# facebookresearch/NasRec

Hardware: AMD Instinct MI355X
Metric: supernet samples/sec at batch 256 (Criteo-shape), 1/2/4/8 MI355X (higher is better)
Workload: dtype f32

## Files before the change

include/nasrec_hip.h:

```cpp
#ifndef NASREC_HIP_H
#define NASREC_HIP_H

#include <stdint.h>

#ifdef __cplusplus
extern "C" {
#endif

#define NASREC_MAX_SEGS 8
#define NASREC_MAX_TABLES 32
#define NASREC_EMB_DIM 16
#define NASREC_MHA_PARAMS 1696
#define NASREC_MHA_SAVED 36

enum {
  NASREC_AM_KC = 0,
  NASREC_AM_RC = 1,
  NASREC_AM_TOKR = 2,
  NASREC_AM_TOKK = 3
};
enum { NASREC_CM_PLAIN = 0,
       NASREC_CM_TOKJ = 1    };
enum { NASREC_ACT_NONE = 0, NASREC_ACT_RELU = 1, NASREC_ACT_SILU = 2, NASREC_ACT_SIGMOID = 3 };

// ... 566 lines not shown
typedef struct nasrec_act_bwd_desc {
  int32_t kind;
  int32_t mode, R, D;
  int32_t ld_dy, ld_z, ld_dz;
  int32_t act, dims_in_use;
  const float* dy;
  const float* z;
  float* dz;
} nasrec_act_bwd_desc_t;

typedef struct nasrec_stage_desc {
  int32_t kind;
  int32_t B, Fd, Fs;
  float lr;
  int32_t _pad;
  const float* int_src;   float* int_dst;
  const int64_t* cat_src; int64_t* cat_dst;
  const float* y_src;     float* y_dst;
  float* lr_dst;
  nasrec_embed_desc_t gather;
  nasrec_dedup_ids_desc_t dedup_ids;
} nasrec_stage_desc_t;

#define NASREC_WL_MAX_ITEMS 12
#define NASREC_WL_BLOB_BYTES 3680
#define NASREC_WL_REDUCE_DST 16
typedef struct nasrec_wl_item {
  int32_t kind, part, off;
  int32_t first, nblk;
  int32_t geom[3];
} nasrec_wl_item_t;

typedef struct nasrec_wl_reduce {
  int32_t kind, R, C, ld;
  const float* in;
  int32_t ndst, _pad;
  float* dst[NASREC_WL_REDUCE_DST];
  int32_t dst_off[NASREC_WL_REDUCE_DST], dst_len[NASREC_WL_REDUCE_DST];
} nasrec_wl_reduce_t;

typedef struct nasrec_worklist_desc {
  int32_t kind;
  int32_t n;
  int32_t total_blocks;
  int32_t _pad;
  nasrec_wl_item_t item[NASREC_WL_MAX_ITEMS];
  char blob[NASREC_WL_BLOB_BYTES] __attribute__((aligned(16)));
} nasrec_worklist_desc_t;

typedef struct nasrec_worklist_dev_desc {
  int32_t kind;
  int32_t total_blocks;
  int32_t big;
  int32_t _pad;
  uint32_t pf[6], pm[6];
  const nasrec_worklist_desc_t* dev;
} nasrec_worklist_dev_desc_t;
int nasrec_worklist_prepare(const nasrec_worklist_desc_t* w, void* dev_buf, nasrec_worklist_dev_desc_t* out);

enum {
  NASREC_WL_BODY_KIND = 0,
  NASREC_WL_BODY_TILE = 1,
  NASREC_WL_BODY_SECOND_PASS = 2,
  NASREC_WL_BODY_DENSE_SMALL = 3,
  NASREC_WL_BODY_DENSE_SMALL_DX = 4,
  NASREC_WL_BODY_TOKEN_FWD = 5,
  NASREC_WL_BODY_TOKEN_DX = 6
};
typedef struct nasrec_wl_geometry {
  int32_t nblk;
  int32_t geom[3];
  int32_t big;
  int32_t body;
} nasrec_wl_geometry_t;
int nasrec_worklist_item_geometry(int kind, int part, const void* desc, int bytes, nasrec_wl_geometry_t* out);
int nasrec_worklist_set_wide_min(int wide_min);

#define NASREC_PS_MAX_DEPS 8
#define NASREC_PS_REPL 16
#define NASREC_PS_SHARDS 8
#define NASREC_PS_COUNTER_STRIDE 16
#define NASREC_PS_FLAG_STRIDE 32
typedef struct nasrec_persist_item {
  int32_t kind, part, off;
  int32_t first, nblk;
  int32_t geom[3];
  int32_t ndeps;
  int32_t deps[NASREC_PS_MAX_DEPS];
  int32_t _pad[3];
} nasrec_persist_item_t;
// ... 88 lines not shown
```

nasrec_amd/_lib.py:

```python
import ctypes as C
import os

import torch

_HERE = os.path.dirname(os.path.abspath(__file__))
LIB_PATH = os.environ.get("NASREC_HIP_LIB") or os.path.join(_HERE, "lib", "libnasrec_hip.so")

MAX_SEGS = 8
MAX_TABLES = 32
FINAL_HEAD_K, FINAL_HEAD_N = 32, 256
EMB_DIM = 16
MHA_PARAMS = 1696
MHA_SAVED = 36
REDUCE_MAX_DST = 48

AM_KC, AM_RC, AM_TOKR, AM_TOKK = 0, 1, 2, 3
CM_PLAIN, CM_TOKJ = 0, 1
ACT_NONE, ACT_RELU, ACT_SILU, ACT_SIGMOID = 0, 1, 2, 3
TSV_OK, TSV_NEEDS_PYTHON, TSV_BAD_COLUMNS = 0, 1, 2
ACT_BY_NAME = {"identity": ACT_NONE, "relu": ACT_RELU, "silu": ACT_SILU}

(OP_GEMM, OP_EMBED_GATHER, OP_DOT_TRI_FWD, OP_DOT_TRI_BWD, OP_FM_FWD, OP_FM_BWD, OP_MHA_FWD, OP_MHA_BWD, OP_REDUCE_ROWS,
 OP_COPY_SEGS, OP_GATE_BWD, OP_ROWSUM, OP_FINAL_FWD, OP_BCE, OP_FINAL_BWD, OP_EMB_DEDUP, OP_SUMSQ, OP_CLIP_COEF,
 OP_ADAGRAD_DENSE, OP_ADAGRAD_ROWS, OP_MEMSET, OP_LAYERNORM_FWD, OP_LAYERNORM_BWD, OP_ADD_SEGS, OP_SCALE,
# ... 168 lines not shown
    _fields_ = [("kind", i32), ("B", i32), ("Fs", i32), ("cap", i32), ("idx", vp), ("leader", vp), ("order", vp), ("lists", vp), ("counts", vp),
                ("heads", vp)]


class OptReduce2Desc(C.Structure):
    _fields_ = [("kind", i32), ("B", i32), ("Fs", i32), ("cap", i32), ("rank_B", i32), ("row_blocks", i32), ("rank_stride", i64), ("rows", vp),
                ("leader", vp), ("order", vp), ("lists", vp), ("counts", vp), ("heads", vp), ("sumsq_partial", vp), ("sumsq", SumsqDesc)]


class StageDesc(C.Structure):
    _fields_ = [("kind", i32), ("B", i32), ("Fd", i32), ("Fs", i32), ("lr", f32), ("_pad", i32), ("int_src", vp), ("int_dst", vp),
                ("cat_src", vp), ("cat_dst", vp), ("y_src", vp), ("y_dst", vp), ("lr_dst", vp), ("gather", EmbedDesc), ("dedup_ids", DedupIdsDesc)]


class OptReduceDesc(C.Structure):
    _fields_ = [("kind", i32), ("_pad", i32), ("dedup", EmbDedupDesc), ("sumsq", SumsqDesc)]


class OptApplyDesc(C.Structure):
    _fields_ = [("kind", i32), ("dense_blocks", i32), ("clip", ClipCoefDesc), ("dense", AdagradDenseDesc), ("rows", AdagradRowsDesc)]


WL_MAX_ITEMS, WL_BLOB_BYTES, WL_REDUCE_DST = 12, 3680, 16
WL_WHOLE, WL_MAIN, WL_EPI = 0, 1, 2


class WlItem(C.Structure):
    _fields_ = [("kind", i32), ("part", i32), ("off", i32), ("first", i32), ("nblk", i32), ("geom", i32 * 3)]


class WlReduce(C.Structure):
    _fields_ = [("kind", i32), ("R", i32), ("C", i32), ("ld", i32), ("in_", vp), ("ndst", i32), ("_pad", i32), ("dst", vp * WL_REDUCE_DST),
                ("dst_off", i32 * WL_REDUCE_DST), ("dst_len", i32 * WL_REDUCE_DST)]


class WorklistDesc(C.Structure):
    _fields_ = [("kind", i32), ("n", i32), ("total_blocks", i32), ("_pad", i32), ("item", WlItem * WL_MAX_ITEMS),
                ("blob", C.c_char * WL_BLOB_BYTES)]


(WL_BODY_KIND, WL_BODY_TILE, WL_BODY_SECOND_PASS, WL_BODY_DENSE_SMALL, WL_BODY_DENSE_SMALL_DX, WL_BODY_TOKEN_FWD,
 WL_BODY_TOKEN_DX) = range(7)


class WlGeometry(C.Structure):
    _fields_ = [("nblk", i32), ("geom", i32 * 3), ("big", i32), ("body", i32)]


class WorklistDevDesc(C.Structure):
    _fields_ = [("kind", i32), ("total_blocks", i32), ("big", i32), ("_pad", i32), ("pf", C.c_uint32 * 6), ("pm", C.c_uint32 * 6), ("dev", vp)]


PS_MAX_DEPS, PS_REPL, PS_SHARDS, PS_COUNTER_STRIDE, PS_FLAG_STRIDE = 8, 16, 8, 16, 32


class PersistItem(C.Structure):
    _fields_ = [("kind", i32), ("part", i32), ("off", i32), ("first", i32), ("nblk", i32), ("geom", i32 * 3), ("ndeps", i32),
                ("deps", i32 * PS_MAX_DEPS), ("_pad", i32 * 3)]


class PersistDesc(C.Structure):
    _fields_ = [("kind", i32), ("n", i32), ("total_blocks", i32), ("blob_bytes", i32), ("items", vp), ("blob", vp), ("chunk_item", vp),
                ("counters", vp), ("flags", vp), ("err", vp), ("chunk_cap", i32), ("big", i32), ("trace", vp), ("host_items", vp), ("host_blob", vp)]


# ... 101 lines not shown
    lib.nasrec_worklist_prepare.argtypes = [vp, vp, vp]
    lib.nasrec_worklist_item_geometry.argtypes = [C.c_int, C.c_int, C.c_char_p, C.c_int, C.POINTER(WlGeometry)]
    lib.nasrec_worklist_set_wide_min.argtypes = [C.c_int]
    lib.nasrec_tsv_parse.argtypes = [vp, i64, i32, i32, vp, i64, vp, vp, vp, C.POINTER(i64), C.POINTER(i32)]
    lib.nasrec_tsv_parse.restype = i64
    for name in ("nasrec_gemm", "nasrec_embedding_gather", "nasrec_embedding_dedup", "nasrec_dot_tri", "nasrec_fm",
                 "nasrec_mha_ffn", "nasrec_layernorm", "nasrec_final_logit", "nasrec_bce_logits", "nasrec_adagrad_dense",
                 "nasrec_adagrad_rows", "nasrec_opt_reduce", "nasrec_opt_apply", "nasrec_worklist", "nasrec_dedup_ids", "nasrec_opt_reduce2", "nasrec_final_fused", "nasrec_weight_decay",
                 "nasrec_opt_moments", "nasrec_last_layer_step", "nasrec_roc_auc", "nasrec_weight_ema", "nasrec_decoupled_decay"):
        getattr(lib, name).argtypes = [vp, vp]
    lib.nasrec_roc_auc_workspace_bytes.argtypes = [i64]
    lib.nasrec_roc_auc_workspace_bytes.restype = i64
    lib.nasrec_gemm_route.argtypes = [vp, C.POINTER(C.c_uint)]
    if lib.nasrec_abi_version() != 17:
        raise EngineError("ABI version mismatch: library %d, binding 17" % lib.nasrec_abi_version())
    sizes = (i32 * 45)()
    n = lib.nasrec_desc_sizes(sizes, 45)
    for kind, cls in DESC_BY_KIND.items():
        if kind >= n or sizes[kind] != C.sizeof(cls):
            raise EngineError("struct layout mismatch for op kind %d: library %d bytes, binding %d bytes"
                              % (kind, sizes[kind] if kind < n else -1, C.sizeof(cls)))
    if n <= 37 or sizes[37] != C.sizeof(PersistItem):
        raise EngineError("struct layout mismatch for nasrec_persist_item_t: library %d bytes, binding %d bytes" % (sizes[37] if n > 37 else -1, C.sizeof(PersistItem)))
    _lib = lib
    return lib


def check(rc):
    if rc != 0:
        raise EngineError("nasrec engine error %d: %s" % (rc, _lib.nasrec_last_error().decode(errors="replace")))
```

nasrec_amd/csrc/worklist.hip:

```cpp
#include <stdlib.h>
#include <string.h>

#include <vector>

#include "worklist_body.h"

#define WL_WIDE_MIN_DEFAULT 700
static int& wl_wide_min() {
  static int v = getenv("NASREC_WL_WIDE_MIN") ? atoi(getenv("NASREC_WL_WIDE_MIN")) : WL_WIDE_MIN_DEFAULT;
  return v;
}
extern "C" int nasrec_worklist_set_wide_min(int wide_min) {
  const int prev = wl_wide_min();
  wl_wide_min() = wide_min;
  return prev;
}

static int wl_gemm_geometry(const nasrec_gemm_desc_t* g, nasrec_wl_item_t& it, int blob_left) {
  if (blob_left < (int)offsetof(nasrec_gemm_desc_t, seg)) return nasrec_set_error(-2, "worklist: gemm descriptor head runs past the blob");
  if (g->nseg < 1 || g->nseg > NASREC_MAX_SEGS) return nasrec_set_error(-2, "worklist: gemm nseg=%d", g->nseg);
  const int need = (int)offsetof(nasrec_gemm_desc_t, seg) + g->nseg * (int)sizeof(nasrec_gemm_seg_t);
  if (need > blob_left) return nasrec_set_error(-2, "worklist: truncated gemm descriptor (%d bytes) runs past the blob", need);
  const int nprob = g->zmode ? g->nseg : 1;
  const int S = g->splitk > 1 ? g->splitk : 1;
  if (g->splitk == NASREC_SPLITK_BALANCED) return nasrec_set_error(-2, "worklist: the balanced schedule is a throughput-regime launch");
  if ((it.part == 0) != (S == 1)) return nasrec_set_error(-2, "worklist: gemm part %d with splitk %d", it.part, g->splitk);
  if (S > 1 && !g->workspace) return nasrec_set_error(-3, "worklist: splitk=%d needs a workspace", S);
  int Mmax = 0, Nmax = 0, Kmax = 0;
  long wgs = 0;
  bool aux = false, uniform = true;
  for (int q = 0; q < nprob; ++q) {
    Mmax = g->seg[q].M > Mmax ? g->seg[q].M : Mmax;
    Nmax = g->seg[q].N > Nmax ? g->seg[q].N : Nmax;
    wgs += (long)((g->seg[q].M + 63) / 64) * ((g->seg[q].N + 63) / 64) * S;
  }
  for (int q = 0; q < g->nseg; ++q) {
    const nasrec_gemm_seg_t& s = g->seg[q];
    if (s.A && s.K > Kmax) Kmax = s.K;
    aux = aux || s.Aaux || s.Baux;
    if (!g->zmode && (s.ones_col != g->seg[0].ones_col || s.Mvalid != g->seg[0].Mvalid)) uniform = false;
    if (!g->zmode && s.A && ((s.Aaux != nullptr) != (g->seg[0].Aaux != nullptr) || (s.Baux != nullptr) != (g->seg[0].Baux != nullptr))) uniform = false;
  }
  if (!uniform) return nasrec_set_error(-2, "worklist: k-segments that disagree on row predicates / mask operands take the plain template");
  {
    const bool kca = g->amode == NASREC_AM_KC || g->amode == NASREC_AM_TOKK, kcb = g->bmode == NASREC_AM_KC || g->bmode == NASREC_AM_TOKK;
    if (!kca && kcb) return nasrec_set_error(-2, "worklist: operand binding a=%d b=%d has no body", g->amode, g->bmode);
  }
  if (Mmax <= 0 || Nmax <= 0) {
// ... 480 lines not shown
        if (tid == 0) o2 = __hip_atomic_fetch_add(cnt + NASREC_PS_SHARDS * NASREC_PS_COUNTER_STRIDE, 1ull, __ATOMIC_RELAXED, __HIP_MEMORY_SCOPE_AGENT);
        o2 = ((unsigned long long)__builtin_amdgcn_readfirstlane((unsigned)(o2 >> 32)) << 32) | (unsigned)__builtin_amdgcn_readfirstlane((unsigned)o2);
        last = (o2 + 1) % (unsigned long long)NS == 0;
      }
      if (last && nsucc > 0 && tid < NASREC_PS_REPL)
        __hip_atomic_store(flags + ((size_t)k * NASREC_PS_REPL + tid) * NASREC_PS_FLAG_STRIDE, e1, __ATOMIC_RELAXED, __HIP_MEMORY_SCOPE_AGENT);
    }
  }
  if (trace && tid == 0) trace[4 * (size_t)bid + 3] = wall_clock64();
}

int nasrec_persist_prepare(nasrec_persist_desc_t* d) {
  if (!d || d->kind != NASREC_OP_PERSIST) return nasrec_set_error(-1, "persist: wrong descriptor kind");
  if (d->n < 1 || d->n > 65535) return nasrec_set_error(-2, "persist: n=%d items", d->n);
  if (!d->host_items || !d->host_blob) return nasrec_set_error(-2, "persist: a host table pointer is null");
  const bool dry = !d->items;
  if (!dry && (!d->blob || !d->chunk_item || !d->counters || !d->flags || !d->err)) return nasrec_set_error(-2, "persist: a device table pointer is null");
  std::vector<nasrec_persist_item_t> tab(d->host_items, d->host_items + d->n);
  bool big = false;
  int first = 0;
  for (int k = 0; k < d->n; ++k) {
    nasrec_persist_item_t& p = tab[k];
    if (p.off < 0 || (p.off & 15) || p.off >= d->blob_bytes) return nasrec_set_error(-2, "persist: item %d offset %d", k, p.off);
    if (p.ndeps < 0 || p.ndeps > NASREC_PS_MAX_DEPS) return nasrec_set_error(-2, "persist: item %d has %d dependencies", k, p.ndeps);
    for (int q = 0; q < p.ndeps; ++q)
      if (p.deps[q] < 0 || p.deps[q] >= k) return nasrec_set_error(-2, "persist: item %d depends on item %d (not an earlier one)", k, p.deps[q]);
    nasrec_wl_item_t w;
    w.kind = p.kind, w.part = p.part, w.off = p.off;
    const int rc = wl_item_geometry(w, d->host_blob + p.off, d->blob_bytes - p.off, k, big);
    if (rc) return rc;
    if (w.nblk < 1) return nasrec_set_error(-2, "persist: item %d (kind %d) has no workgroups; the caller drops empty operators", k, p.kind);
    static const int max_wg = getenv("NASREC_PS_MAX_WG") ? atoi(getenv("NASREC_PS_MAX_WG")) : 512;
    const bool tiles = p.kind == NASREC_OP_GEMM && p.part != 2 && (w.geom[2] & 3) != WL_TOKS;
    const bool walks = (p.kind == NASREC_OP_GEMM && p.part == 2) || p.kind == NASREC_OP_FINAL_BWD || tiles;
    const int hint = d->host_items[k]._pad[1];
    const int cap = hint > 0 ? hint : (tiles ? 1 << 30 : max_wg);
    const int upw = walks ? (w.nblk + cap - 1) / (cap > 0 ? cap : 1) : 1;
    const int nwg = (w.nblk + upw - 1) / upw;
    p.first = first, p.nblk = w.nblk;
    p.geom[0] = w.geom[0], p.geom[1] = w.geom[1], p.geom[2] = w.geom[2];
    p._pad[1] = nwg;
    p._pad[2] = ((k + 1 < d->n ? d->host_items[k + 1].off : d->blob_bytes) - p.off + 63) & ~63;
    first += nwg;
  }
  for (int k = 0; k < d->n; ++k) tab[k]._pad[0] = 0;
  for (int k = 0; k < d->n; ++k)
// ... 37 lines not shown
```

nasrec_amd/csrc/worklist_body.h:

```cpp
#pragma once
#include "attention_tok.h"
#include "gemm_rt.h"
#include "final_bodies.h"
#include "interact_bodies.h"
#include "dedup_bodies.h"

#define WL_LDS_BIG_FLOATS 9888
#define WL_LDS_FLOATS 7840
static_assert(MHA_TOK_BWD_LDS_FLOATS <= WL_LDS_BIG_FLOATS && MHA_TOK_FWD_LDS_FLOATS <= WL_LDS_FLOATS, "Transformer bodies fit the worklist launches");

#define WL_TK 64
#ifndef WL_AUX_RING2
#define WL_AUX_RING2 0
#endif
enum { WL_TOKS = 0, WL_T32x32 = 1, WL_T64x16 = 2, WL_T16x64 = 3 };
#define WL_WIDE 32
#define WL_WIDE_TK 32

extern __shared__ __attribute__((aligned(16))) float wl_lds[];

template <typename T>
__device__ __forceinline__ const T& wl_ref(unsigned long long addr) {
  const unsigned lo = __builtin_amdgcn_readfirstlane((unsigned)addr), hi = __builtin_amdgcn_readfirstlane((unsigned)(addr >> 32));
  return *(const T*)(const __attribute__((address_space(4))) T*)(((unsigned long long)hi << 32) | lo);
// ... 306 lines not shown
      for (int j = 0; j < 4; ++j) fx[s][j] = xb[min(16 * s + 4 * fg + j, K - 1) * 16];
#pragma unroll
    for (int s = 0; s < WL_TOKDX_STEPS; ++s)
#pragma unroll
      for (int j = 0; j < 4; ++j) fb[s][j] = fx[s][j] > 0.f ? fb[s][j] : 0.f;
  }
  f32x4 acc = {0.f, 0.f, 0.f, 0.f};
#pragma unroll
  for (int s = 0; s < WL_TOKDX_STEPS; ++s) {
    if (16 * s < K) {
#pragma unroll
      for (int j = 0; j < 4; ++j) {
        const bool in = 16 * s + 4 * fg + j < K;
        acc = __builtin_amdgcn_mfma_f32_16x16x4f32(in ? fa[s][j] : 0.f, in ? fb[s][j] : 0.f, acc, 0, 0, 0);
      }
    }
  }
  {
    const float v4[4] = {acc[0], acc[1], acc[2], acc[3]};
    if (t * 16 + 4 * fg < M) epilogue_store_col4<NASREC_CM_TOKJ>(g, sg, t * 16 + 4 * fg, b * 16 + e, M, v4);
  }
}

__device__ __forceinline__ void wl_gemm_second_pass(unsigned long long blob, int vb_, int per_) {
  const nasrec_gemm_desc_t& g = wl_ref<nasrec_gemm_desc_t>(blob);
  const int vb = __builtin_amdgcn_readfirstlane(vb_), per = __builtin_amdgcn_readfirstlane(per_);
  const int nprob = g.zmode ? g.nseg : 1;
  int Mmax = 0, Nmax = 0;
  for (int q = 0; q < nprob; ++q) {
    Mmax = max(Mmax, g.seg[q].M);
    Nmax = max(Nmax, g.seg[q].N);
  }
  int z = vb / per, v = vb - z * per;
  if (WL_COMPACT_Z && g.zmode) {
    z = 0, v = vb;
    for (; z < nprob - 1; ++z) {
      const int cnt = wl_z_units(g.seg[z].M, g.seg[z].N);
      if (v < cnt) break;
      v -= cnt;
    }
  }
  const long e = (long)v * 256 + threadIdx.x;
  if (g.cmode == NASREC_CM_PLAIN)
    splitk_second_pass<NASREC_CM_PLAIN>(g, Mmax, Nmax, z, e);
  else
    splitk_second_pass<NASREC_CM_TOKJ>(g, Mmax, Nmax, z, e);
}

__device__ __forceinline__ void wl_mha_fwd(unsigned long long blob, int vb) {
  mha_fwd_tok(wl_ref<nasrec_mha_desc_t>(blob), __builtin_amdgcn_readfirstlane(vb), wl_lds);
}

#define WL_PACKED_NONE 0xffffffffu
#define WL_HEAD_BYTES 48
static inline int wl_item_body(int kind, int part, const int32_t (&geom)[3]) {
  if (kind != NASREC_OP_GEMM) return NASREC_WL_BODY_KIND;
  if (part == 2) return NASREC_WL_BODY_SECOND_PASS;
  const int cfg = geom[2];
  if ((cfg & 3) != WL_TOKS) return NASREC_WL_BODY_TILE;
  if (((cfg >> 2) & 3) == 3) return geom[1] == 0 ? NASREC_WL_BODY_DENSE_SMALL_DX : NASREC_WL_BODY_DENSE_SMALL;
  return ((cfg >> 2) & 3) == 1 ? NASREC_WL_BODY_TOKEN_FWD : NASREC_WL_BODY_TOKEN_DX;
}
template <bool BIG>
__device__ __forceinline__ void wl_run(unsigned f01, unsigned f23, unsigned f45, unsigned f67, unsigned f89, unsigned fab, unsigned m01, unsigned m23,
                                       unsigned m45, unsigned m67, unsigned m89, unsigned mab, const unsigned long long base) {
  const nasrec_worklist_desc_t& wl = wl_ref<nasrec_worklist_desc_t>(base);
  float* lds = wl_lds;
  const int bid = blockIdx.x, tid = threadIdx.x, wave = tid >> 6, lane = tid & 63;
  int k = 0, it_first = 0, it_kind, it_part, it_off;
  if (f01 != WL_PACKED_NONE) {
    const unsigned f[6] = {f01, f23, f45, f67, f89, fab}, m[6] = {m01, m23, m45, m67, m89, mab};
    unsigned meta = m01 & 0xffffu;
#pragma unroll
    for (int q = 1; q < NASREC_WL_MAX_ITEMS; ++q) {
      const unsigned fq = (f[q >> 1] >> (16 * (q & 1))) & 0xffffu, mq = (m[q >> 1] >> (16 * (q & 1))) & 0xffffu;
      if ((unsigned)bid >= fq) {
        k = q;
        it_first = (int)fq;
        meta = mq;
      }
    }
    it_kind = meta & 63;
    it_part = (meta >> 6) & 3;
    it_off = (int)(meta >> 8) * 16;
  } else {
#pragma unroll 1
    while (k + 1 < wl.n && bid >= wl.item[k + 1].first) ++k;
    it_first = wl.item[k].first;
    it_kind = wl.item[k].kind;
    it_part = wl.item[k].part;
    it_off = wl.item[k].off;
  }
  const nasrec_wl_item_t& it = wl.item[k];
  const int vb = bid - it_first;
  const unsigned long long blob = base + offsetof(nasrec_worklist_desc_t, blob) + it_off;
  switch (it_kind) {
    case NASREC_OP_GEMM: {
      if (it_part == 2) {
        wl_gemm_second_pass(blob, vb, it.geom[0]);
        break;
      }
      const int cfg = it.geom[2];
      if ((cfg & 3) == WL_TOKS && ((cfg >> 2) & 3) == 3 && it.geom[1] == 0) wl_dense_small_dx(blob, vb, it.geom[0]);
      else if ((cfg & 3) == WL_TOKS && ((cfg >> 2) & 3) == 3) wl_dense_small(blob, vb, it.geom[0], it.geom[1]);
      else if ((cfg & 3) == WL_TOKS && ((cfg >> 2) & 3) == 1) wl_token_fwd(blob, vb, it.geom[0]);
      else if ((cfg & 3) == WL_TOKS) wl_token_dx(blob, vb, it.geom[0]);
      else if ((cfg >> 4) & 1) wl_gemm_bind<true>((cfg >> 2) & 3, cfg & 3, blob, vb, it.geom[0], it.geom[1]);
      else wl_gemm_bind<false>((cfg >> 2) & 3, cfg & (3 | WL_WIDE), blob, vb, it.geom[0], it.geom[1]);
      break;
    }
    case NASREC_OP_MHA_FWD:
      wl_mha_fwd(blob, vb);
      break;
    case NASREC_OP_MHA_BWD:
      if (BIG) mha_bwd_tok(wl_ref<nasrec_mha_desc_t>(blob), __builtin_amdgcn_readfirstlane(vb), wl_lds);
      break;
    case NASREC_OP_FM_FWD: {
      const nasrec_fm_desc_t& d = wl_ref<nasrec_fm_desc_t>(blob);
      const int b = vb * 4 + wave;
      if (b < d.B) fm_fwd_sample(d, b, lane);
      break;
    }
    case NASREC_OP_FM_BWD: {
      const nasrec_fm_desc_t& d = wl_ref<nasrec_fm_desc_t>(blob);
// ... 63 lines not shown
```

nasrec_amd/engine.py:

```python
import copy
import ctypes as C
import json
import math
import os
from typing import Dict, List, Optional

import torch

from . import _lib as L
from . import plan as P
from . import schedule as S
from .optim_spec import OptimSpec

E = 16
DEDUP_SPLIT_MAX_B = min(int(os.environ.get("NASREC_DEDUP_SPLIT_MAX_B", "2048")), L.DEDUP_IDS_MAX_B)
_IDS_AS_ITEM = os.environ.get("NASREC_IDS_AS_ITEM", "1") != "0"
_WL_TUNE = os.environ.get("NASREC_WL_TUNE", "0") == "1"
_WL_TUNE_MARGIN = float(os.environ.get("NASREC_WL_TUNE_MARGIN", "0.004"))
_WL_RESIDENT = os.environ.get("NASREC_WL_RESIDENT", "1") != "0"
_FUSE_FINAL = os.environ.get("NASREC_FUSE_FINAL", "1") != "0"
_FIXED_OPT_TABLE = os.environ.get("NASREC_FIXED_OPT_TABLE", "1") != "0"


def _ptr_array(descs):
# ... 397 lines not shown
            w = ctx.param("_final.weight", (1, K))
            bptr = ctx.param("_final.bias", (1,))
            fd = L.FinalDesc()
            fd.kind = L.OP_FINAL_FWD
            fd.B, fd.nseg = B, len(fsegs)
            fd.w, fd.bias, fd.logits = w, bptr, cp.logits.data_ptr()
            for q, (s, ts) in enumerate(fsegs):
                fd.seg[q], fd.width[q], fd.ld[q], fd.off[q], fd.tok_stride[q] = s.view.ptr, s.width, s.view.ld, s.koff, ts
            ctx.emit(fd)
            if cfg.use_final_sigmoid:
                raise NotImplementedError("use_final_sigmoid is never enabled by the reference CLIs")
            scheduled = self.level_schedule and cfg.fixed and B <= 256
            cp.fwd_levels = cp.bwd_levels = None
            cp.dead_forward = []
            if train:
                if not spec.moments or spec.table_kind:
                    self._ensure_table_state()
                self._build_training_tail(cp, ctx, w, bptr, fsegs, B, K, grad_scale)
            fwd_list = list(ctx.fwd)
            if self.dead_code_elimination and cfg.fixed:
                fwd_list, cp.dead_forward = S.eliminate_dead_forward(fwd_list, ctx.bwd if train else [])
            if scheduled:
                fwd_list = S.order_two_term_accumulates(fwd_list)
                fwd_descs, cp.fwd_levels = S.pack(fwd_list)
                self._resident_worklists(cp, fwd_descs)
            else:
                fwd_descs = fwd_list
            cp.fwd = Program(fwd_descs)
            cp.used_params = list(ctx.used_params)
            if train:
                bd, pre = cp.bce, cp._pre
                fi = next(i for i, dsc in enumerate(ctx.bwd) if isinstance(dsc, L.FinalDesc))
                plain = ctx.bwd[fi]
                assert plain.kind == L.OP_FINAL_BWD
                fused = L.FinalDesc.from_buffer_copy(plain)
                fused.logits, fused.y, fused.loss, fused.dlogits_out = cp.logits.data_ptr(), cp.y.data_ptr(), cp.loss.data_ptr(), cp.dlogits.data_ptr()
                fused.grad_scale = bd.grad_scale
                cp.bce = bd
                bwd_descs = pre[1:] + ctx.bwd[:fi] + [fused] + ctx.bwd[fi + 1:]
                odescs = []
                cp.ids_on_stage = False
                if local_optimizer:
                    odescs = self._optimizer_descs(cp.tail, B, cp.cat_x, sbuf.grad_tensor() if (sbuf.grad_written and not self.host_embedding)
                                                   else None, clip, eps)
                cp.decay0 = cp.tail.decay0 if (local_optimizer and spec.dwd) else None
                ids_in_program = []
                ids = cp.tail.dedup_ids
# ... 5 lines not shown
                        cp.ids_on_stage = True
                    else:
                        odescs = [ids] + odescs
                cp.fb = None
                if scheduled:
                    jf, jb = self._fuse_final(fwd_list, bwd_descs, fused) if _FUSE_FINAL else (fwd_list, bwd_descs)
                    jf, jb = self._fuse_head(jf, jb)
                    fb_descs = None
                    cp.persistent = False
                    cp.level_tuning = None
                    if persist:
                        try:
                            if spec.ema:
                                raise S.PersistRefused("a weight-EMA plan keeps the default launches")
                            fb_descs, cp.fb_levels = S.pack_persistent(
                                ids_in_program + jf + jb, lambda nb: torch.empty(max(int(nb), 16), dtype=torch.uint8, device=self.device),
                                arena.ranges, alloc=ctx.alloc)
                            cp.persistent = True
                            self._persist_errs += [d.err_tensor for d in fb_descs if isinstance(d, L.PersistDesc)]
                        except S.PersistRefused as e:
                            import warnings
                            warnings.warn("persistent step refused (%s): one launch per level instead" % (e,))
                    if fb_descs is None:
                        fb_descs, cp.fb_levels = S.pack(ids_in_program + jf + jb, alloc=ctx.alloc)
                        if _WL_TUNE and S.BALANCE:
                            fb_descs, cp.level_tuning = self._tune_levels(ids_in_program + jf + jb, ctx.alloc, fb_descs)
                    self._resident_worklists(cp, fb_descs)
                    cp.fb = Program(fb_descs)
                    bwd_descs, cp.bwd_levels = S.pack(bwd_descs)
                    self._resident_worklists(cp, bwd_descs)
                cp.bwd = Program(bwd_descs)
                cp.bwd_tail_start = len(pre) - 1 + ctx.bwd_tail_start
                cp.bwd_marks = [(b, len(pre) - 1 + idx) for b, idx in ctx.block_marks]
                cp.bwd_core = Program(pre[1:] + ctx.bwd)
                last = L.FinalDesc.from_buffer_copy(plain)
                for q in range(L.MAX_SEGS):
                    last.dseg[q] = None
                tail = [ctx.bwd[fi + 1]] if plain.nsplit > 1 else []
                cp.bwd_final_only = Program(pre[1:] + [last] + tail)
                cp.opt = Program(odescs)
                if graph:
                    cp.step = Program((cp.fb.descs if cp.fb is not None else cp.fwd.descs + cp.bwd.descs) + cp.opt.descs)
                    cp.step.capture(self.stream.cuda_stream)
            elif graph:
                cp.fwd.capture(self.stream.cuda_stream)
        cp.bf16_launches = P.bf16_launches(cp.fwd.descs) + (P.bf16_launches(cp.bwd.descs) if train else 0)
        cp.bf16_token_launches = P.bf16_token_launches(cp.fwd.descs) + (P.bf16_token_launches(cp.bwd.descs) if train else 0)
        if graph or arena is None or cfg.fixed:
            self.stream.synchronize()
        self._plans[key] = cp
        self._last_plan = (fast, choice, cp)
        return cp
# ... 1022 lines not shown
```

nasrec_amd/schedule.py:

```python
import ctypes as C
import os
from typing import List, Tuple

from . import _lib as L

E = 16
MHA_PARAM_FLOATS = [768, 48, 256, 16, 16, 16, 256, 16, 256, 16, 16, 16]


class Acc:
    __slots__ = ("ptr", "width", "stride", "rows", "end")

    def __init__(self, ptr, rows, width_f, ld_f):
        self.ptr = int(ptr)
        self.rows = max(int(rows), 1)
        self.width = int(width_f) * 4
        self.stride = int(ld_f) * 4 if self.rows > 1 else self.width
        if self.stride < self.width:
            self.stride = self.width
        self.end = self.ptr + (self.rows - 1) * self.stride + self.width


def _flat(ptr, n_floats):
    return Acc(ptr, 1, n_floats, n_floats)
# ... 10 lines not shown


def _operand(ptr, mode, R, K, ld):
    if not ptr:
        return None
    if mode == L.AM_KC:
        return Acc(ptr, R, K, ld)
    if mode == L.AM_RC:
        return Acc(ptr, K, R, ld)
    if mode == L.AM_TOKR:
        return Acc(ptr, (R + 15) // 16, K * E, ld)
    return Acc(ptr, (K + 15) // 16, R * E, ld)


def _cview(ptr, cmode, M, N, ldc):
    if not ptr:
        return None
    if cmode == L.CM_PLAIN:
        return Acc(ptr, M, N, ldc)
    return Acc(ptr, (N + 15) // 16, M * E, ldc)


def _gemm_io(d, part):
    R, W = [], []
    nprob = d.nseg if d.zmode else 1
    S = d.splitk if d.splitk > 1 else 1
    Mm = max(d.seg[q].M for q in range(nprob))
    Nm = max(d.seg[q].N for q in range(nprob))
    ws = _flat(d.workspace, S * Mm * Nm * nprob) if (S > 1 and d.workspace) else None
    if d.splitk == L.SPLITK_BALANCED and d.workspace:
        ws = _flat(d.workspace, L.SK_WORKSPACE_FLOATS)
    if part in ("whole", "main"):
        for q in range(d.nseg):
            s = d.seg[q]
            if not s.A:
                continue
            M, N = (s.M, s.N) if d.zmode else (d.seg[0].M, d.seg[0].N)
            Nb = N - (1 if s.ones_col else 0)
            for ptr, mode, rr, ld in ((s.A, d.amode, M, s.lda), (s.Aaux, d.amode, M, s.lda), (s.B, d.bmode, Nb, s.ldb), (s.Baux, d.bmode, Nb, s.ldb)):
                a = _operand(ptr, mode, rr, s.K, ld)
                if a is not None:
                    R.append(a)
        if part == "main":
            W.append(ws)
            return R, W
        if part == "whole" and ws is not None:
# ... 193 lines not shown

    def __init__(self, desc, part="whole"):
        self.desc, self.part = desc, part
        self.level = 0
        self.index = 0

    def __getattr__(self, name):
        if name in ("reads", "writes"):
            io = desc_io(self.desc, self.part)
            self.reads, self.writes = io if io is not None else (None, None)
        elif name == "item":
            self.item = _item(self)
        else:
            raise AttributeError(name)
        return getattr(self, name)


def expand(descs, cut=lambda d: not d.defer_second_pass) -> List[Node]:
    nodes = []
    for d in descs:
        if isinstance(d, L.GemmDesc) and d.splitk > 1 and cut(d):
            nodes.append(Node(d, "main"))
            nodes.append(Node(d, "epi"))
        else:
            nodes.append(Node(d))
    for i, n in enumerate(nodes):
        n.index = i
    return nodes


def expand_for_worklists(descs) -> List[Node]:
    return expand(descs, gemm_capable)


def _depends(later: Node, earlier: Node) -> bool:
    if later.reads is None or earlier.reads is None:
        return True
    for w in earlier.writes:
        for a in later.reads:
            if overlap(w, a):
                return True
        for a in later.writes:
            if overlap(w, a):
                return True
    for r in earlier.reads:
        for a in later.writes:
# ... 207 lines not shown
        if not (plain(Q) and Q.beta == 1 and Q.cmode == P.cmode and (sq.C, sq.M, sq.N, sq.ldc) == (sp.C, sp.M, sp.N, sp.ldc)):
            continue
        between = range(ip + 1, iq)
        if any(overlap(r, c) for i in between for r in nodes[i].reads):
            continue
        if not any(_depends(nodes[iq], nodes[i]) for i in between):
            up = True
        elif not any(_depends(nodes[i], nodes[ip]) for i in between):
            up = False
        else:
            continue
        ready_q = max([nodes[j].level + 1 for j in range(iq) if j != ip and _depends(nodes[iq], nodes[j])] + [0])
        if ready_q >= nodes[ip].level:
            continue
        first, second = _copy_desc(Q), _copy_desc(P)
        first.beta, second.beta = 0, 1
        out = list(fwd)
        rest = [fwd[i] for i in between]
        out[ip:iq + 1] = [first, second] + rest if up else rest + [first, second]
        return order_two_term_accumulates(out)
    return fwd


_GEMM_HEAD = L.GemmDesc.seg.offset
_SEG_BYTES = C.sizeof(L.GemmSeg)
_PART = {"whole": L.WL_WHOLE, "main": L.WL_MAIN, "epi": L.WL_EPI}


def item_geometry(kind, part, b):
    g = L.WlGeometry()
    return g if L.load().nasrec_worklist_item_geometry(kind, _PART[part], b, len(b), C.byref(g)) == 0 else None


SOLO_TILES = int(os.environ.get("NASREC_WL_SOLO_TILES", "256"))


def _gemm_bytes(d):
    return C.string_at(C.addressof(d), _GEMM_HEAD + d.nseg * _SEG_BYTES)


def _gemm_wanted(d) -> bool:
    if d.defer_second_pass or d.nseg < 1 or d.nseg > L.MAX_SEGS:
        return False
    nprob = d.nseg if d.zmode else 1
    S = d.splitk if d.splitk > 1 else 1
    if nprob == 1 and ((d.seg[0].M + 63) // 64) * ((d.seg[0].N + 63) // 64) * S >= SOLO_TILES:
        return False
    if not getattr(d, "_wl_force", False):
        from . import plan as P
        one = d
        if d.splitk > 1:
            one = L.GemmDesc.from_buffer_copy(d)
            one.splitk = 1
        if P.gemm_route(one)[1] & (1 << L.GEMM_ROUTE_KSLICE):
            return False
    return True


def gemm_capable(d) -> bool:
    return _gemm_wanted(d) and item_geometry(d.kind, "whole" if d.splitk <= 1 else "main", _gemm_bytes(d)) is not None


def _item(node):
    d = node.desc
    if isinstance(d, L.GemmDesc):
        if not _gemm_wanted(d):
            return None
        b = _gemm_bytes(d)
    elif d.kind == L.OP_REDUCE_ROWS and d.ndst <= L.WL_REDUCE_DST:
        r = L.WlReduce()
        r.kind, r.R, r.C, r.ld, r.in_, r.ndst = d.kind, d.R, d.C, d.ld, d.in_, d.ndst
        for q in range(d.ndst):
            r.dst[q], r.dst_off[q], r.dst_len[q] = d.dst[q], d.dst_off[q], d.dst_len[q]
        b = C.string_at(C.addressof(r), C.sizeof(r))
    else:
        b = C.string_at(C.addressof(d), C.sizeof(d))
    g = item_geometry(d.kind, node.part, b)
    return (b, g) if g is not None else None


def item_bytes(node):
    return node.item[0] if node.item is not None else None


_ITEM_NS = {L.OP_MHA_BWD: 18000, L.OP_MHA_FWD: 11000, L.OP_DOT_TRI_BWD: 10000, L.OP_DOT_TRI_FWD: 6000, L.OP_REDUCE_ROWS: 4500,
            L.OP_FM_BWD: 3900, L.OP_FM_FWD: 3500, L.OP_FINAL_BWD: 7500, L.OP_DEDUP_IDS: 8000, L.OP_FINAL_FUSED: 4500}
_ITEM_NS_R4 = {L.OP_MHA_BWD: 18500, L.OP_MHA_FWD: 10500, L.OP_REDUCE_ROWS: 6000, L.OP_FM_BWD: 7000, L.OP_FM_FWD: 3500, L.OP_FINAL_BWD: 7000,
               L.OP_FINAL_FWD: 3400, L.OP_GATE_BWD: 3500, L.OP_DEDUP_IDS: 8000, L.OP_FINAL_FUSED: 4500}
_COST_MODEL = os.environ.get("NASREC_WL_COST", "time")
# ... 48 lines not shown

def _item_beats_kernel(d):
    if not (_SOLO_ITEMS and isinstance(d, L.GemmDesc) and d.splitk <= 1 and 1 <= d.nseg <= L.MAX_SEGS):
        return False
    g = item_geometry(d.kind, "whole", _gemm_bytes(d))
    return g is not None and g.body == L.WL_BODY_TOKEN_DX


def pack(descs, alloc=None):
    if BALANCE and RESPLIT and alloc is not None:
        descs = resplit_slack_solos(descs, alloc)
    nodes = expand_for_worklists(descs)
    nl = assign_levels(nodes)
    if BALANCE:
        balance_levels(nodes, nl)
    out = []
    for lv in range(nl):
        members = sorted((n for n in nodes if n.level == lv), key=lambda n: -_cost(n))
        solo, items = [], []
        for n in members:
            b = item_bytes(n)
            (items if b is not None else solo).append((n, b))
        for n, _ in solo:
            assert n.part == "whole"
            out.append(n.desc)
        if len(items) == 1 and items[0][0].part == "whole" and not _item_beats_kernel(items[0][0].desc):
            out.append(items[0][0].desc)
            continue
        cur, off = None, 0
        for n, b in items:
            size = (len(b) + 15) & ~15
            if cur is None or cur.n == L.WL_MAX_ITEMS or off + size > L.WL_BLOB_BYTES:
                cur = L.WorklistDesc()
                cur.kind, cur.n = L.OP_WORKLIST, 0
                cur.nodes = []
                off = 0
                out.append(cur)
            it = cur.item[cur.n]
            it.kind, it.part, it.off = n.desc.kind, _PART[n.part], off
            C.memmove(C.addressof(cur) + L.WorklistDesc.blob.offset + off, b, len(b))
            cur.n += 1
            cur.nodes.append(n)
            off += size
    return out, nl


PERSIST = os.environ.get("NASREC_PERSIST", "1") != "0"
# ... 154 lines not shown
```

Baseline: 1.192 million.

## Chain accumulating token-axis input-gradient GEMMs into one worklist item

Measured after the change: 1.233 million, median of 6. +3.5%, better.

```diff
diff --git a/include/nasrec_hip.h b/include/nasrec_hip.h
--- a/include/nasrec_hip.h
+++ b/include/nasrec_hip.h
@@ -612,6 +612,7 @@
   nasrec_dedup_ids_desc_t dedup_ids;
 } nasrec_stage_desc_t;
 
+#define NASREC_WL_CHAIN 3
 #define NASREC_WL_MAX_ITEMS 12
 #define NASREC_WL_BLOB_BYTES 3680
 #define NASREC_WL_REDUCE_DST 16
@@ -655,7 +656,8 @@
   NASREC_WL_BODY_DENSE_SMALL = 3,
   NASREC_WL_BODY_DENSE_SMALL_DX = 4,
   NASREC_WL_BODY_TOKEN_FWD = 5,
-  NASREC_WL_BODY_TOKEN_DX = 6
+  NASREC_WL_BODY_TOKEN_DX = 6,
+  NASREC_WL_BODY_TOKEN_DX_CHAIN = 7
 };
 typedef struct nasrec_wl_geometry {
   int32_t nblk;
diff --git a/nasrec_amd/_lib.py b/nasrec_amd/_lib.py
--- a/nasrec_amd/_lib.py
+++ b/nasrec_amd/_lib.py
@@ -214,7 +214,7 @@
 
 
 WL_MAX_ITEMS, WL_BLOB_BYTES, WL_REDUCE_DST = 12, 3680, 16
-WL_WHOLE, WL_MAIN, WL_EPI = 0, 1, 2
+WL_WHOLE, WL_MAIN, WL_EPI, WL_CHAIN = 0, 1, 2, 3
 
 
 class WlItem(C.Structure):
@@ -232,7 +232,7 @@
 
 
 (WL_BODY_KIND, WL_BODY_TILE, WL_BODY_SECOND_PASS, WL_BODY_DENSE_SMALL, WL_BODY_DENSE_SMALL_DX, WL_BODY_TOKEN_FWD,
- WL_BODY_TOKEN_DX) = range(7)
+ WL_BODY_TOKEN_DX, WL_BODY_TOKEN_DX_CHAIN) = range(8)
 
 
 class WlGeometry(C.Structure):
@@ -380,8 +380,20 @@
                               % (kind, sizes[kind] if kind < n else -1, C.sizeof(cls)))
     if n <= 37 or sizes[37] != C.sizeof(PersistItem):
         raise EngineError("struct layout mismatch for nasrec_persist_item_t: library %d bytes, binding %d bytes" % (sizes[37] if n > 37 else -1, C.sizeof(PersistItem)))
+    g, probe = WlGeometry(), _chain_probe()
+    if lib.nasrec_worklist_item_geometry(OP_GEMM, WL_CHAIN, probe, len(probe), C.byref(g)) != 0 or (g.nblk, g.geom[0], g.geom[1], g.body) != (1, 1, 1, WL_BODY_TOKEN_DX_CHAIN):
+        raise EngineError("the library does not know the chained worklist item (part %d): rebuild it" % WL_CHAIN)
     _lib = lib
     return lib
+
+
+def _chain_probe():
+    d = GemmDesc()
+    d.kind, d.amode, d.bmode, d.cmode, d.nseg, d.zmode, d.dims_in_use = OP_GEMM, AM_RC, AM_TOKR, CM_TOKJ, 2, 1, -1
+    for q in range(2):
+        s = d.seg[q]
+        s.A, s.B, s.C, s.M, s.N, s.K, s.lda, s.ldb, s.ldc, s.accumulate = 64, 64, 64, 16, 16, 16, 16, 256, 256, q
+    return C.string_at(C.addressof(d), GemmDesc.seg.offset + 2 * C.sizeof(GemmSeg))
 
 
 def check(rc):
diff --git a/nasrec_amd/csrc/worklist.hip b/nasrec_amd/csrc/worklist.hip
--- a/nasrec_amd/csrc/worklist.hip
+++ b/nasrec_amd/csrc/worklist.hip
@@ -14,6 +14,36 @@
   const int prev = wl_wide_min();
   wl_wide_min() = wide_min;
   return prev;
+}
+
+static int wl_chain_geometry(const nasrec_gemm_desc_t* g, nasrec_wl_item_t& it) {
+  if (!g->zmode || g->amode != NASREC_AM_RC || g->bmode != NASREC_AM_TOKR || g->cmode != NASREC_CM_TOKJ)
+    return nasrec_set_error(-2, "worklist: a chained item is a zmode token-axis input gradient (a=%d b=%d c=%d zmode=%d)", g->amode, g->bmode, g->cmode, g->zmode);
+  if (g->splitk > 1) return nasrec_set_error(-2, "worklist: a chained item is unsplit (splitk=%d)", g->splitk);
+  if (g->bias || g->act != NASREC_ACT_NONE || g->dims_in_use >= 0 || g->pre_add || g->mul_nseg != 0 || g->save_z || g->save_act)
+    return nasrec_set_error(-2, "worklist: a chained item has a plain epilogue (no bias, activation, mask, residual, gate or saved copy)");
+  if (!g->seg[0].C) return nasrec_set_error(-2, "worklist: chained item without an output");
+  int h = 0;
+  for (int q = 1; q < g->nseg && !h; ++q)
+    if (g->seg[q].C == g->seg[0].C) h = q;
+  if (h < 1 || g->nseg % h != 0) return nasrec_set_error(-2, "worklist: chained item of %d problems: no second writer of the first output, or chains of unequal length", g->nseg);
+  const int N = g->seg[0].N;
+  if (N <= 0 || (N & 15)) return nasrec_set_error(-2, "worklist: chained item with N=%d (whole samples of 16 columns)", N);
+  int TU = 0;
+  for (int q = 0; q < g->nseg; ++q) {
+    const nasrec_gemm_seg_t &s = g->seg[q], &s0 = g->seg[q % h];
+    if (s.Aaux || s.ones_col || (s.Mvalid > 0 && s.Mvalid < s.M)) return nasrec_set_error(-2, "worklist: chained problem %d has a weight mask, a ones column or a row predicate", q);
+    if (s.K > 16 * WL_TOKDX_STEPS) return nasrec_set_error(-2, "worklist: chained problem %d has K=%d > %d", q, s.K, 16 * WL_TOKDX_STEPS);
+    if (s.M <= 0 || s.N != N) return nasrec_set_error(-2, "worklist: chained problem %d is %d x %d (N=%d everywhere)", q, s.M, s.N, N);
+    if (s.C != s0.C || s.M != s0.M || s.ldc != s0.ldc) return nasrec_set_error(-2, "worklist: chained problem %d does not write what problem %d writes", q, q % h);
+    if (q >= h && !s.accumulate) return nasrec_set_error(-2, "worklist: chained problem %d overwrites the sum of its predecessors", q);
+    if (q < h) TU += (s.M + 15) / 16;
+  }
+  it.geom[0] = TU;
+  it.geom[1] = h;
+  it.geom[2] = WL_TOKS | (2 << 2);
+  it.nblk = std::min(((N >> 4) * TU + 3) / 4, WL_TOK_MAX_WG);
+  return 0;
 }
 
 static int wl_gemm_geometry(const nasrec_gemm_desc_t* g, nasrec_wl_item_t& it, int blob_left) {
@@ -24,6 +54,7 @@
   const int nprob = g->zmode ? g->nseg : 1;
   const int S = g->splitk > 1 ? g->splitk : 1;
   if (g->splitk == NASREC_SPLITK_BALANCED) return nasrec_set_error(-2, "worklist: the balanced schedule is a throughput-regime launch");
+  if (it.part == NASREC_WL_CHAIN) return wl_chain_geometry(g, it);
   if ((it.part == 0) != (S == 1)) return nasrec_set_error(-2, "worklist: gemm part %d with splitk %d", it.part, g->splitk);
   if (S > 1 && !g->workspace) return nasrec_set_error(-3, "worklist: splitk=%d needs a workspace", S);
   int Mmax = 0, Nmax = 0, Kmax = 0;
@@ -550,6 +581,7 @@
   for (int k = 0; k < d->n; ++k) {
     nasrec_persist_item_t& p = tab[k];
     if (p.off < 0 || (p.off & 15) || p.off >= d->blob_bytes) return nasrec_set_error(-2, "persist: item %d offset %d", k, p.off);
+    if (p.kind == NASREC_OP_GEMM && p.part == NASREC_WL_CHAIN) return nasrec_set_error(-2, "persist: item %d is a chained product; the persistent form takes the unchained program", k);
     if (p.ndeps < 0 || p.ndeps > NASREC_PS_MAX_DEPS) return nasrec_set_error(-2, "persist: item %d has %d dependencies", k, p.ndeps);
     for (int q = 0; q < p.ndeps; ++q)
       if (p.deps[q] < 0 || p.deps[q] >= k) return nasrec_set_error(-2, "persist: item %d depends on item %d (not an earlier one)", k, p.deps[q]);
diff --git a/nasrec_amd/csrc/worklist_body.h b/nasrec_amd/csrc/worklist_body.h
--- a/nasrec_amd/csrc/worklist_body.h
+++ b/nasrec_amd/csrc/worklist_body.h
@@ -352,6 +352,94 @@
   }
 }
 
+__device__ __forceinline__ void wl_token_dx_chain_unit(const nasrec_gemm_desc_t& g, int unit, int TU, int h, int c, int e, int fg) {
+  const int b = unit / TU;
+  int t = unit - b * TU, q = 0;
+  while (q < h - 1 && t >= ((g.seg[q].M + 15) >> 4)) t -= (g.seg[q].M + 15) >> 4, ++q;
+  const nasrec_gemm_seg_t& s0 = g.seg[q];
+  const int M = s0.M, ldc = s0.ldc, i0 = t * 16 + 4 * fg;
+  const int row = min(t * 16 + e, M - 1);
+  float* const Cp = s0.C;
+  long o[4];
+#pragma unroll
+  for (int r = 0; r < 4; ++r) o[r] = c_offset<NASREC_CM_TOKJ>(min(i0 + r, M - 1), b * 16 + e, ldc);
+  float v[4] = {0.f, 0.f, 0.f, 0.f};
+  if (s0.accumulate) {
+#pragma unroll
+    for (int r = 0; r < 4; ++r) v[r] = Cp[o[r]];
+  }
+  for (int m = 0; m < c; m += 2) {
+    float fa[2][WL_TOKDX_STEPS][4], fb[2][WL_TOKDX_STEPS][4];
+    int K2[2];
+#pragma unroll
+    for (int u = 0; u < 2; ++u) {
+      const nasrec_gemm_seg_t& sg = g.seg[q + min(m + u, c - 1) * h];
+      const bool live = m + u < c && sg.A != nullptr && sg.K > 0;
+      const int K = live ? sg.K : 0;
+      K2[u] = K;
+      if (live) {
+        const float* wp = sg.A + row;
+        const float* yb = sg.B + (long)b * sg.ldb + e;
+#pragma unroll
+        for (int s = 0; s < WL_TOKDX_STEPS; ++s)
+#pragma unroll
+          for (int j = 0; j < 4; ++j) {
+            const int k = min(16 * s + 4 * fg + j, K - 1);
+            fa[u][s][j] = wp[(long)k * sg.lda];
+            fb[u][s][j] = yb[k * 16];
+          }
+      }
+    }
+#pragma unroll
+    for (int u = 0; u < 2; ++u) {
+      const nasrec_gemm_seg_t& sg = g.seg[q + min(m + u, c - 1) * h];
+      const int K = K2[u];
+      if (K > 0 && sg.Baux) {
+        const float* xb = sg.Baux + (long)b * sg.ldb + e;
+        float fx[WL_TOKDX_STEPS][4];
+#pragma unroll
+        for (int s = 0; s < WL_TOKDX_STEPS; ++s)
+#pragma unroll
+          for (int j = 0; j < 4; ++j) fx[s][j] = xb[min(16 * s + 4 * fg + j, K - 1) * 16];
+#pragma unroll
+        for (int s = 0; s < WL_TOKDX_STEPS; ++s)
+#pragma unroll
+          for (int j = 0; j < 4; ++j) fb[u][s][j] = fx[s][j] > 0.f ? fb[u][s][j] : 0.f;
+      }
+    }
+#pragma unroll
+    for (int u = 0; u < 2; ++u) {
+      const int K = K2[u];
+      if (K <= 0) continue;
+      f32x4 acc = {0.f, 0.f, 0.f, 0.f};
+#pragma unroll
+      for (int s = 0; s < WL_TOKDX_STEPS; ++s) {
+        if (16 * s < K) {
+#pragma unroll
+          for (int j = 0; j < 4; ++j) {
+            const bool in = 16 * s + 4 * fg + j < K;
+            acc = __builtin_amdgcn_mfma_f32_16x16x4f32(in ? fa[u][s][j] : 0.f, in ? fb[u][s][j] : 0.f, acc, 0, 0, 0);
+          }
+        }
+      }
+      const bool over = m + u == 0 && !s0.accumulate;
+#pragma unroll
+      for (int r = 0; r < 4; ++r) v[r] = over ? acc[r] : acc[r] + v[r];
+    }
+  }
+#pragma unroll
+  for (int r = 0; r < 4; ++r)
+    if (i0 + r < M) Cp[o[r]] = v[r];
+}
+__device__ __forceinline__ void wl_token_dx_chain(unsigned long long blob, int vb_, int TU_, int h_) {
+  const nasrec_gemm_desc_t& g = wl_ref<nasrec_gemm_desc_t>(blob);
+  const int vb = __builtin_amdgcn_readfirstlane(vb_), TU = __builtin_amdgcn_readfirstlane(TU_), h = __builtin_amdgcn_readfirstlane(h_);
+  const int lane = threadIdx.x & 63, wave = __builtin_amdgcn_readfirstlane(threadIdx.x >> 6);
+  wl_warm_blob(blob, (int)offsetof(nasrec_gemm_desc_t, seg) + g.nseg * (int)sizeof(nasrec_gemm_seg_t));
+  const int total = (g.seg[0].N >> 4) * TU, stride = 4 * min((total + 3) >> 2, WL_TOK_MAX_WG);
+  for (int unit = vb * 4 + wave; unit < total; unit += stride) wl_token_dx_chain_unit(g, unit, TU, h, g.nseg / h, lane & 15, lane >> 4);
+}
+
 __device__ __forceinline__ void wl_gemm_second_pass(unsigned long long blob, int vb_, int per_) {
   const nasrec_gemm_desc_t& g = wl_ref<nasrec_gemm_desc_t>(blob);
   const int vb = __builtin_amdgcn_readfirstlane(vb_), per = __builtin_amdgcn_readfirstlane(per_);
@@ -386,6 +474,7 @@
 static inline int wl_item_body(int kind, int part, const int32_t (&geom)[3]) {
   if (kind != NASREC_OP_GEMM) return NASREC_WL_BODY_KIND;
   if (part == 2) return NASREC_WL_BODY_SECOND_PASS;
+  if (part == NASREC_WL_CHAIN) return NASREC_WL_BODY_TOKEN_DX_CHAIN;
   const int cfg = geom[2];
   if ((cfg & 3) != WL_TOKS) return NASREC_WL_BODY_TILE;
   if (((cfg >> 2) & 3) == 3) return geom[1] == 0 ? NASREC_WL_BODY_DENSE_SMALL_DX : NASREC_WL_BODY_DENSE_SMALL;
@@ -430,6 +519,10 @@
         wl_gemm_second_pass(blob, vb, it.geom[0]);
         break;
       }
+      if (it_part == NASREC_WL_CHAIN) {
+        wl_token_dx_chain(blob, vb, it.geom[0], it.geom[1]);
+        break;
+      }
       const int cfg = it.geom[2];
       if ((cfg & 3) == WL_TOKS && ((cfg >> 2) & 3) == 3 && it.geom[1] == 0) wl_dense_small_dx(blob, vb, it.geom[0]);
       else if ((cfg & 3) == WL_TOKS && ((cfg >> 2) & 3) == 3) wl_dense_small(blob, vb, it.geom[0], it.geom[1]);
diff --git a/nasrec_amd/engine.py b/nasrec_amd/engine.py
--- a/nasrec_amd/engine.py
+++ b/nasrec_amd/engine.py
@@ -443,7 +443,7 @@
                 fwd_list, cp.dead_forward = S.eliminate_dead_forward(fwd_list, ctx.bwd if train else [])
             if scheduled:
                 fwd_list = S.order_two_term_accumulates(fwd_list)
-                fwd_descs, cp.fwd_levels = S.pack(fwd_list)
+                fwd_descs, cp.fwd_levels = S.pack(S.chain_accumulates(fwd_list))
                 self._resident_worklists(cp, fwd_descs)
             else:
                 fwd_descs = fwd_list
@@ -495,12 +495,13 @@
                             import warnings
                             warnings.warn("persistent step refused (%s): one launch per level instead" % (e,))
                     if fb_descs is None:
-                        fb_descs, cp.fb_levels = S.pack(ids_in_program + jf + jb, alloc=ctx.alloc)
+                        joint = S.chain_accumulates(ids_in_program + jf + jb)
+                        fb_descs, cp.fb_levels = S.pack(joint, alloc=ctx.alloc)
                         if _WL_TUNE and S.BALANCE:
-                            fb_descs, cp.level_tuning = self._tune_levels(ids_in_program + jf + jb, ctx.alloc, fb_descs)
+                            fb_descs, cp.level_tuning = self._tune_levels(joint, ctx.alloc, fb_descs)
                     self._resident_worklists(cp, fb_descs)
                     cp.fb = Program(fb_descs)
-                    bwd_descs, cp.bwd_levels = S.pack(bwd_descs)
+                    bwd_descs, cp.bwd_levels = S.pack(S.chain_accumulates(bwd_descs))
                     self._resident_worklists(cp, bwd_descs)
                 cp.bwd = Program(bwd_descs)
                 cp.bwd_tail_start = len(pre) - 1 + ctx.bwd_tail_start
diff --git a/nasrec_amd/schedule.py b/nasrec_amd/schedule.py
--- a/nasrec_amd/schedule.py
+++ b/nasrec_amd/schedule.py
@@ -56,6 +56,8 @@
 
 
 def _gemm_io(d, part):
+    if part == "chain":
+        part = "whole"
     R, W = [], []
     nprob = d.nseg if d.zmode else 1
     S = d.splitk if d.splitk > 1 else 1
@@ -295,6 +297,8 @@
         if isinstance(d, L.GemmDesc) and d.splitk > 1 and cut(d):
             nodes.append(Node(d, "main"))
             nodes.append(Node(d, "epi"))
+        elif getattr(d, "_chain", 0):
+            nodes.append(Node(d, "chain"))
         else:
             nodes.append(Node(d))
     for i, n in enumerate(nodes):
@@ -548,9 +552,78 @@
     return fwd
 
 
+CHAIN = os.environ.get("NASREC_WL_CHAIN", "1") != "0"
+_CHAIN_HEAD = ("amode", "bmode", "cmode", "zmode", "act", "dims_in_use", "splitk", "defer_second_pass", "bias", "save_z", "save_act", "mul_nseg",
+               "pre_add", "bias_on_rows", "mask_on_rows")
+
+
+def _merged_chain(P, Q):
+    h = getattr(P, "_chain", 0) or P.nseg
+    if Q.nseg != h or P.nseg + h > L.MAX_SEGS or any(getattr(P, f) != getattr(Q, f) for f in _CHAIN_HEAD):
+        return None
+    for q in range(h):
+        p, s = P.seg[q], Q.seg[q]
+        if not s.C or (s.C, s.M, s.N, s.ldc) != (p.C, p.M, p.N, p.ldc) or not s.accumulate:
+            return None
+    m = _copy_desc(P)
+    for q in range(h):
+        m.seg[P.nseg + q] = Q.seg[q]
+    m.nseg = P.nseg + h
+    m._chain = h
+    m._chain_of = getattr(P, "_chain_of", (P,)) + (Q,)
+    return m if item_geometry(m.kind, "chain", _gemm_bytes(m)) is not None else None
+
+
+def chain_accumulates(descs):
+    if not CHAIN:
+        return descs
+    nodes = expand_for_worklists(descs)
+    assign_levels(nodes)
+
+    def candidate(n):
+        d = n.desc
+        return (n.part in ("whole", "chain") and isinstance(d, L.GemmDesc) and d.zmode and d.splitk <= 1 and n.reads is not None
+                and 1 <= d.nseg <= L.MAX_SEGS)
+
+    for ip, p in enumerate(nodes):
+        if not candidate(p):
+            continue
+        P = p.desc
+        h = getattr(P, "_chain", 0) or P.nseg
+        cs = [c for c in (_cview(P.seg[q].C, P.cmode, P.seg[q].M, P.seg[q].N, P.seg[q].ldc) for q in range(h)) if c is not None]
+        if len(cs) != h:
+            continue
+        iq = next((i for i in range(ip + 1, len(nodes))
+                   if nodes[i].reads is None or any(overlap(a, c) for c in cs for a in nodes[i].reads + nodes[i].writes)), None)
+        if iq is None or nodes[iq].part != "whole" or not candidate(nodes[iq]):
+            continue
+        q = nodes[iq]
+        between = range(ip + 1, iq)
+        if not any(_depends(q, nodes[i]) for i in between):
+            up = True
+        elif not any(_depends(nodes[i], p) for i in between):
+            up = False
+        else:
+            continue
+        ready_q = max([nodes[j].level + 1 for j in range(iq) if j != ip and _depends(q, nodes[j])] + [0])
+        if ready_q > p.level:
+            continue
+        if p.part == "whole" and (p.item is None or p.item[1].body != L.WL_BODY_TOKEN_DX):
+            continue
+        if q.item is None or q.item[1].body != L.WL_BODY_TOKEN_DX:
+            continue
+        m = _merged_chain(P, q.desc)
+        if m is None:
+            continue
+        out = [d for d in descs if d is not (q.desc if up else P)]
+        out[next(k for k, d in enumerate(out) if d is (P if up else q.desc))] = m
+        return chain_accumulates(out)
+    return descs
+
+
 _GEMM_HEAD = L.GemmDesc.seg.offset
 _SEG_BYTES = C.sizeof(L.GemmSeg)
-_PART = {"whole": L.WL_WHOLE, "main": L.WL_MAIN, "epi": L.WL_EPI}
+_PART = {"whole": L.WL_WHOLE, "main": L.WL_MAIN, "epi": L.WL_EPI, "chain": L.WL_CHAIN}
 
 
 def item_geometry(kind, part, b):
@@ -590,7 +663,7 @@
 def _item(node):
     d = node.desc
     if isinstance(d, L.GemmDesc):
-        if not _gemm_wanted(d):
+        if node.part != "chain" and not _gemm_wanted(d):
             return None
         b = _gemm_bytes(d)
     elif d.kind == L.OP_REDUCE_ROWS and d.ndst <= L.WL_REDUCE_DST:
@@ -685,7 +758,7 @@
             b = item_bytes(n)
             (items if b is not None else solo).append((n, b))
         for n, _ in solo:
-            assert n.part == "whole"
+            assert n.part == "whole", n.part
             out.append(n.desc)
         if len(items) == 1 and items[0][0].part == "whole" and not _item_beats_kernel(items[0][0].desc):
             out.append(items[0][0].desc)
```
